# trzy/FasterRCNN

Hardware: AMD Instinct MI355X
Metric: images/sec (600x1000) Faster-RCNN VGG-16 inference (higher is better)
Workload: dtype f32 (float32 tensors and accumulation; 15 GEMM layers in the f32x3 split-operand emulation = two fp16 terms per block-scaled operand, three fp16 MFMAs per product; 0 in f32x6 = three bf16 terms, six bf16 MFMAs; the other 2 on exact-f32 MFMA; strict exact-f32 everywhere: config.strict_f32_images_per_

## Files before the change

### fasterrcnn_amd/_native.py

```python
import ctypes as C
import os

_HERE = os.path.dirname(os.path.abspath(__file__))
LIB_PATH = os.environ.get("FRCNN_LIB_PATH") or os.path.join(_HERE, "csrc", "libfrcnn_hip.so")

OK = 0
ABI_VERSION = 21
ERRORS = {0: "FRCNN_OK", -1: "FRCNN_EINVAL", -2: "FRCNN_EHIP", -3: "FRCNN_ENOMEM",
          -4: "FRCNN_EUNSUPPORTED", -5: "FRCNN_ENODEVICE"}
RELU = 1
POOL2 = 2
NUM_KCLASS = 11
KCLASS_NAMES = ("conv3x3_mfma", "conv3x3_c3", "linear_mfma", "proposals", "roi_pool", "other", "winograd_transforms",
                "winograd_gemm", "winograd_x6_transforms", "winograd_x6_gemm", "winograd_x3f")

SYMBOLS = (
    "frcnn_abi_version", "frcnn_error_string", "frcnn_last_hip_error", "frcnn_device_count",
    "frcnn_anchors", "frcnn_pack_conv3x3", "frcnn_pack_conv3x3_c3", "frcnn_pack_fc_chw_to_hwc",
    "frcnn_pack_stack_rows", "frcnn_conv3x3_c3", "frcnn_conv3x3_c3_cmax", "frcnn_conv3x3_workspace_bytes", "frcnn_conv3x3_nhwc",
    "frcnn_maxpool2x2_nhwc",
    "frcnn_linear_workspace_bytes", "frcnn_linear", "frcnn_softmax_rows", "frcnn_rpn_proposals",
    "frcnn_nms", "frcnn_roi_pool", "frcnn_roi_pool_x3t", "frcnn_detections", "frcnn_ctx_create", "frcnn_ctx_create_proposals", "frcnn_ctx_destroy",
    "frcnn_ctx_bytes", "frcnn_vgg16_forward", "frcnn_ctx_tensor", "frcnn_ctx_timing_enable",
    "frcnn_ctx_timing_read",
    "frcnn_fold_bn_pack", "frcnn_conv_workspace_bytes", "frcnn_conv_nhwc", "frcnn_conv_nhwc_math", "frcnn_conv_nhwc_x3g", "frcnn_conv_nhwc_x3g_tickets", "frcnn_pack_conv_x3g_weights", "frcnn_x3_saturation_events", "frcnn_tensor_absmax", "frcnn_conv7x7_s2_c3",
    "frcnn_maxpool3x3_s2_nhwc", "frcnn_spatial_mean_nhwc", "frcnn_resnet_forward", "frcnn_rpn_targets",
    "frcnn_preprocess_workspace_bytes", "frcnn_preprocess",
    "frcnn_conv3x3_uses_winograd", "frcnn_resnet_block_uses_winograd", "frcnn_pack_conv3x3_winograd",
    "frcnn_pack_conv3x3_winograd_taps", "frcnn_conv3x3_winograd_workspace_bytes",
    "frcnn_conv3x3_nhwc_winograd",
    "frcnn_conv3x3_uses_winograd_fused", "frcnn_resnet_block_uses_winograd_fused", "frcnn_pack_conv3x3_winograd_fused", "frcnn_pack_conv3x3_winograd_fused_taps",
    "frcnn_conv3x3_nhwc_winograd_fused",
    "frcnn_roi_align", "frcnn_roi_align_backward",
    "frcnn_x6t_record_bytes", "frcnn_split_rows_x6t", "frcnn_gemm_x6t_workspace_bytes", "frcnn_gemm_x6t", "frcnn_split_pixels_x6t", "frcnn_split_patches3x3_x6t",
    "frcnn_conv3x3_uses_winograd_x6", "frcnn_conv3x3_winograd_x6_pack_bytes", "frcnn_pack_conv3x3_winograd_x6",
    "frcnn_conv3x3_winograd_x6_workspace_bytes", "frcnn_conv3x3_nhwc_winograd_x6",
    "frcnn_pixel_absmax", "frcnn_split_pixels_x3t", "frcnn_split_patches3x3_x3t",
    "frcnn_x3t_blob_bytes", "frcnn_pack_rows_x3t", "frcnn_conv3x3_winograd_x3_pack_bytes", "frcnn_pack_conv3x3_winograd_x3",
    "frcnn_conv3x3_winograd_x3_workspace_bytes", "frcnn_conv3x3_nhwc_winograd_x3",
    "frcnn_conv3x3_winograd_x3_fused_workspace_bytes", "frcnn_conv3x3_nhwc_winograd_x3_fused", "frcnn_conv3x3_nhwc_winograd_x3_chain",
    "frcnn_x3t_record_bytes", "frcnn_rows_scale_x3t", "frcnn_split_rows_x3t", "frcnn_gemm_x3t_workspace_bytes", "frcnn_gemm_x3t",
    "frcnn_conv3x3_nhwc_winograd_fused_maps", "frcnn_ctx_create_backbone", "frcnn_resnet_backbone", "frcnn_resnet_forward_features", "frcnn_resnet_rpn_roipool", "frcnn_ctx_create_head", "frcnn_resnet_head",
    "frcnn_label_proposals", "frcnn_gather_rows", "frcnn_rpn_loss", "frcnn_detector_loss",
    "frcnn_gemm_tn_math", "frcnn_conv3x3_wgrad_math", "frcnn_conv_wgrad_math", "frcnn_bottleneck_backward_workspace_bytes", "frcnn_bottleneck_backward",
    "frcnn_gemm_tn_workspace_bytes", "frcnn_gemm_tn", "frcnn_conv3x3_wgrad_workspace_bytes", "frcnn_conv3x3_wgrad",
    "frcnn_pack_conv3x3_dgrad", "frcnn_relu_backward", "frcnn_dropout", "frcnn_dropout_relu_backward", "frcnn_add_inplace", "frcnn_maxpool2x2_backward",
    "frcnn_roi_pool_backward_workspace_bytes", "frcnn_roi_pool_backward", "frcnn_transpose", "frcnn_sgd_step", "frcnn_sgd_step_fold",
    "frcnn_conv_wgrad_workspace_bytes", "frcnn_conv_wgrad", "frcnn_conv_dgrad_workspace_bytes", "frcnn_conv_dgrad", "frcnn_conv_dgrad_math",
    "frcnn_pack_conv_dgrad", "frcnn_scale_rows", "frcnn_bn_scale_shift", "frcnn_spatial_mean_backward",
    "frcnn_ops_roi_align", "frcnn_ops_roi_align_backward", "frcnn_ops_roi_pool", "frcnn_ops_roi_pool_backward",
    "frcnn_ops_nms_workspace_bytes", "frcnn_ops_nms",
    "frcnn_ops_ms_roi_align", "frcnn_ops_ms_roi_align_workspace_bytes", "frcnn_ops_ms_roi_align_backward",
    "frcnn_ops_half_run", "frcnn_ops_roi_align_16", "frcnn_ops_roi_align_backward_16", "frcnn_ops_roi_pool_16",
    "frcnn_ops_roi_pool_backward_16", "frcnn_ops_ms_roi_align_16", "frcnn_ops_ms_roi_align_backward_16",
)


# ... 230 lines not shown
    "frcnn_detector_loss": (C.c_int, [_vp, _vp, _vp, _vp, _i, _i, _vp, _vp, _i, _vp]),
    "frcnn_gemm_tn_workspace_bytes": (C.c_size_t, [_i, _i, _i]),
    "frcnn_gemm_tn": (C.c_int, [_vp, _i, _vp, _i, _vp, _i, _i, _i, _i, _vp, _sz, _vp]),
    "frcnn_gemm_tn_math": (C.c_int, [_vp, _i, _vp, _i, _vp, _i, _i, _i, _i, _i, _vp, _sz, _vp]),
    "frcnn_conv3x3_wgrad_math": (C.c_int, [_vp, _vp, _vp, _i, _i, _i, _i, _i, _vp, _sz, _vp]),
    "frcnn_conv_wgrad_math": (C.c_int, [_vp, _vp, _vp, _i, _i, _i, _i, _i, _i, _i, _i, _i, _vp, _sz, _vp]),
    "frcnn_bottleneck_backward_workspace_bytes": (C.c_int, [_vp, _vp, _vp, _vp, _i, _i, _i, _i, _i, C.POINTER(C.c_size_t), C.POINTER(C.c_size_t)]),
    "frcnn_bottleneck_backward": (C.c_int, [_vp, _vp, _vp, _vp, _vp, _vp, _vp, _vp, _vp, _vp, _vp, _vp, _vp, _i, _i, _i, _i, _i, _i, _vp, _sz, _vp, _sz,
                                            _vp, _vp]),
    "frcnn_conv3x3_wgrad_workspace_bytes": (C.c_size_t, [_i, _i, _i, _i]),
    "frcnn_conv3x3_wgrad": (C.c_int, [_vp, _vp, _vp, _i, _i, _i, _i, _vp, _sz, _vp]),
    "frcnn_pack_conv3x3_dgrad": (C.c_int, [_vp, _vp, _i, _i, _vp]),
    "frcnn_conv_wgrad_workspace_bytes": (C.c_size_t, [_i] * 8),
    "frcnn_conv_wgrad": (C.c_int, [_vp, _vp, _vp, _i, _i, _i, _i, _i, _i, _i, _i, _vp, _sz, _vp]),
    "frcnn_conv_dgrad_workspace_bytes": (C.c_size_t, [_i] * 8),
    "frcnn_conv_dgrad": (C.c_int, [_vp, _vp, _vp, _vp, _i, _i, _i, _i, _i, _i, _i, _i, _vp, _sz, _vp]),
    "frcnn_conv_dgrad_math": (C.c_int, [_vp, _vp, _vp, _vp, _i, _i, _i, _i, _i, _i, _i, _i, _i, _vp, _sz, _vp]),
    "frcnn_pack_conv_dgrad": (C.c_int, [_vp, _vp, _i, _i, _i, _vp]),
    "frcnn_scale_rows": (C.c_int, [_vp, _vp, _vp, _i, _i, _i, _vp]),
    "frcnn_bn_scale_shift": (C.c_int, [_vp, _vp, _vp, _vp, _f, _i, _vp, _vp, _vp]),
    "frcnn_spatial_mean_backward": (C.c_int, [_vp, _vp, _i, _i, _i, _i, _vp]),
    "frcnn_relu_backward": (C.c_int, [_vp, _vp, _sz, _vp]),
    "frcnn_dropout": (C.c_int, [_vp, _sz, _f, _f, _vp, C.c_uint32, C.c_uint32, _vp, _vp]),
    "frcnn_dropout_relu_backward": (C.c_int, [_vp, _vp, _sz, _f, _vp]),
    "frcnn_add_inplace": (C.c_int, [_vp, _vp, _sz, _vp]),
    "frcnn_maxpool2x2_backward": (C.c_int, [_vp, _vp, _vp, _i, _i, _i, _vp]),
    "frcnn_roi_pool_backward_workspace_bytes": (C.c_size_t, [_i, _i, _i]),
    "frcnn_roi_pool_backward": (C.c_int, [_vp, _i, _i, _i, _vp, _i, _i, _f, _vp, _vp, _i, _vp, _sz, _vp]),
    "frcnn_transpose": (C.c_int, [_vp, _i, _vp, _i, _i, _i, _vp]),
    "frcnn_sgd_step": (C.c_int, [_vp, _vp, _vp, _sz, _f, _f, _f, _i, _vp]),
    "frcnn_sgd_step_fold": (C.c_int, [_vp, _vp, _vp, _sz, _f, _f, _f, _i, _vp, _vp, _i, _i, _vp]),
    "frcnn_ctx_timing_enable": (C.c_int, [_vp, _i]),
    "frcnn_ctx_timing_read": (C.c_int, [_vp, C.POINTER(C.c_double), C.POINTER(C.c_int64), _i]),
}


def lib():
    global _lib
    if _lib is not None:
        return _lib
    import torch
    if not os.path.exists(LIB_PATH):
        raise RuntimeError(
            "fasterrcnn_amd: %s is missing. Build it with `python -m fasterrcnn_amd.build` "
            "(hipcc --offload-arch=gfx950). There is no CPU fallback for this path." % LIB_PATH)
    try:
        handle = C.CDLL(LIB_PATH)
    except OSError as e:
        raise RuntimeError("fasterrcnn_amd: cannot load %s: %s" % (LIB_PATH, e)) from e
    for name in SYMBOLS:
        try:
            fn = getattr(handle, name)
        except AttributeError as e:
            raise RuntimeError("fasterrcnn_amd: %s does not export %s (stale build?)" % (LIB_PATH, name)) from e
        restype, argtypes = _SIGNATURES[name]
        fn.restype = restype
        fn.argtypes = argtypes
    if handle.frcnn_abi_version() != ABI_VERSION:
        raise RuntimeError("fasterrcnn_amd: ABI version mismatch in %s" % LIB_PATH)
    _lib = handle
    return _lib


def check(rc, where):
    if rc != OK:
        detail = ""
        if rc == -2:
# ... 30 lines not shown
```

### fasterrcnn_amd/csrc/api.hip

```cpp
#include "common.h"
#include <algorithm>
#include <cmath>
#include <cstring>
#include <string>
#include <vector>
#include <new>

namespace frcnn {

static thread_local std::string g_hip_error;
void set_hip_error(hipError_t e) { g_hip_error = hipGetErrorString(e); }

static size_t align_up(size_t v, size_t a) { return (v + a - 1) / a * a; }

struct EventRec { int cls; hipEvent_t start, stop; };

}

using namespace frcnn;

struct frcnn_ctx {
    int max_h = 0, max_w = 0, max_rois = 0, max_images = 0;
    int max_fh = 0, max_fw = 0, a_cap = 0, pre_cap = 0;
    void* slab = nullptr;
// ... 3 lines not shown
    float *rpn_trunk = nullptr;
    float *rpn_head = nullptr;
    float *scores = nullptr;
    int32_t* sorted_idx = nullptr;
    float *anchor_map = nullptr, *valid_map = nullptr;
    float *roi_out = nullptr;
    float *fc1_out = nullptr, *fc2_out = nullptr;
    void *roi_rec = nullptr, *fc1_rec = nullptr;
    int rec_rows = 0;
    float *roi_inv = nullptr, *fc1_inv = nullptr, *fm_cmax = nullptr;
    float *head_logits = nullptr;
    void* lin_ws = nullptr; size_t lin_ws_bytes = 0;
    void* conv_ws = nullptr; size_t conv_ws_bytes = 0;
    void* wino_ws = nullptr; size_t wino_ws_bytes = 0;
    void* wx_ws = nullptr; size_t wx_ws_bytes = 0;
    int max_head_rois = 0;
    float* x3f_cmax = nullptr; size_t x3f_cmax_bytes = 0;
    void* rx_rec = nullptr; size_t rx_rec_bytes = 0;
    void* rx_ws = nullptr; size_t rx_ws_bytes = 0;
    float* rx_aux = nullptr; size_t rx_aux_floats = 0;
    float* gx_max = nullptr; int gx_next = 0; const float* gx_x = nullptr;
    unsigned* gx_cnt = nullptr;
    float* res_buf[5] = {nullptr, nullptr, nullptr, nullptr, nullptr};
    size_t res_buf_floats = 0;
    int last_c = 512, last_vec = 4096, last_head_ld = 128;
    ProposalScratch ps{};
    int anc_h = -1, anc_w = -1, anc_fh = -1, anc_fw = -1;
    int last_fh = 0, last_fw = 0, last_pre = 0, last_post = 0;
    bool timing = false;
    std::vector<EventRec> recs;
    std::vector<hipEvent_t> free_events;
    double t_ms[FRCNN_NUM_KCLASS] = {0};
    int64_t t_cnt[FRCNN_NUM_KCLASS] = {0};
};

namespace {

struct Scope {
    frcnn_ctx* c; int cls; hipStream_t s; hipEvent_t e0 = nullptr, e1 = nullptr; bool on;
    Scope(frcnn_ctx* c_, int cls_, hipStream_t s_) : c(c_), cls(cls_), s(s_), on(c_ && c_->timing) {
        if (!on) return;
        e0 = take(); e1 = take();
        if (!e0 || !e1) { on = false; return; }
        (void)hipEventRecord(e0, s);
    }
    ~Scope() {
        if (!on) return;
        (void)hipEventRecord(e1, s);
        c->recs.push_back(EventRec{cls, e0, e1});
    }
    hipEvent_t take() {
        if (!c->free_events.empty()) { hipEvent_t e = c->free_events.back(); c->free_events.pop_back(); return e; }
        hipEvent_t e = nullptr;
        if (hipEventCreate(&e) != hipSuccess) return nullptr;
        return e;
    }
};

inline hipStream_t as_stream(void* s) { return reinterpret_cast<hipStream_t>(s); }

}

extern "C" {

int frcnn_abi_version(void) { return FRCNN_ABI_VERSION; }

// ... 899 lines not shown
    unsigned char* p = static_cast<unsigned char*>(c->slab);
    for (auto& it : items) { *it.p = p; p += align_up(it.bytes, 256); }
    c->lin_ws_bytes = lin;
    c->conv_ws_bytes = cws;
    proposal_scratch_carve(c->ps, ps_base, c->a_cap, c->pre_cap, 2048);
    *out = c;
    return FRCNN_OK;
}

int frcnn_ctx_create_proposals(frcnn_ctx** out, int max_image_h, int max_image_w)
{
    if (!out || max_image_h < 16 || max_image_w < 16) return FRCNN_EINVAL;
    frcnn_ctx* c = new (std::nothrow) frcnn_ctx();
    if (!c) return FRCNN_ENOMEM;
    c->max_h = max_image_h; c->max_w = max_image_w; c->max_rois = 0;
    c->max_fh = cdiv(max_image_h, 16); c->max_fw = cdiv(max_image_w, 16);
    c->a_cap = c->max_fh * c->max_fw * 9;
    if (c->a_cap < 16384) c->a_cap = 16384;
    c->pre_cap = 16384;
    const size_t total = align_up(proposal_scratch_bytes(c->a_cap, c->pre_cap, 2048), 256);
    hipError_t e = hipMalloc(&c->slab, total);
    if (e != hipSuccess) { set_hip_error(e); delete c; return FRCNN_ENOMEM; }
    c->slab_bytes = total;
    proposal_scratch_carve(c->ps, c->slab, c->a_cap, c->pre_cap, 2048);
    *out = c;
    return FRCNN_OK;
}

void frcnn_ctx_destroy(frcnn_ctx* ctx)
{
    if (!ctx) return;
    for (auto& r : ctx->recs) { (void)hipEventDestroy(r.start); (void)hipEventDestroy(r.stop); }
    for (auto e : ctx->free_events) (void)hipEventDestroy(e);
    if (ctx->slab) (void)hipFree(ctx->slab);
    if (ctx->wino_ws) (void)hipFree(ctx->wino_ws);
    if (ctx->wx_ws) (void)hipFree(ctx->wx_ws);
    if (ctx->x3f_cmax) (void)hipFree(ctx->x3f_cmax);
    if (ctx->roi_rec) (void)hipFree(ctx->roi_rec);
    if (ctx->rx_rec) (void)hipFree(ctx->rx_rec);
    if (ctx->rx_ws) (void)hipFree(ctx->rx_ws);
    if (ctx->rx_aux) (void)hipFree(ctx->rx_aux);
    if (ctx->gx_max) (void)hipFree(ctx->gx_max);
    if (ctx->gx_cnt) (void)hipFree(ctx->gx_cnt);
    delete ctx;
}

size_t frcnn_ctx_bytes(const frcnn_ctx* ctx) { return ctx ? ctx->slab_bytes + ctx->wino_ws_bytes + ctx->wx_ws_bytes + ctx->rx_rec_bytes + ctx->rx_ws_bytes + (ctx->roi_rec ? (size_t)ctx->rec_rows * (49 * 512 + 4096) * 6 : 0) : 0; }

int frcnn_ctx_timing_enable(frcnn_ctx* ctx, int enable)
{
    if (!ctx) return FRCNN_EINVAL;
    ctx->timing = enable != 0;
    return FRCNN_OK;
}

int frcnn_ctx_timing_read(frcnn_ctx* ctx, double ms[FRCNN_NUM_KCLASS], int64_t launches[FRCNN_NUM_KCLASS], int reset)
{
    if (!ctx || !ms || !launches) return FRCNN_EINVAL;
    for (auto& r : ctx->recs) {
        FRCNN_HIP_TRY(hipEventSynchronize(r.stop));
        float t = 0.f;
        FRCNN_HIP_TRY(hipEventElapsedTime(&t, r.start, r.stop));
        ctx->t_ms[r.cls] += t;
        ctx->t_cnt[r.cls] += 1;
        ctx->free_events.push_back(r.start);
        ctx->free_events.push_back(r.stop);
// ... 715 lines not shown
                const float* d_anchor_map, const float* d_valid_map, float* d_props, float* d_classes, float* d_deltas, int32_t* d_counts,
                hipStream_t s)
{
    int rc = resnet_rpn_roi(c, w, p, H, W, fh, fw, C, d_anchor_map, d_valid_map, d_props, d_counts, c->roi_out, s);
    if (rc) return rc;
    return resnet_head(c, w, p, c->roi_out, p->post_nms, d_classes, d_deltas, s);
}
}

int frcnn_resnet_forward(frcnn_ctx* c, const frcnn_resnet_weights* w, const frcnn_forward_params* p,
                         const float* d_image, int H, int W, const float* d_anchor_map,
                         const float* d_valid_map, float* d_props, float* d_classes, float* d_deltas,
                         int32_t* d_counts, void* stream)
{
    if (!c || !w || !p || !d_image || !d_props || !d_classes || !d_deltas || !d_counts) return FRCNN_EINVAL;
    if (H < 32 || W < 32 || H > c->max_h || W > c->max_w) return FRCNN_EINVAL;
    if (p->post_nms < 1 || p->post_nms > c->max_rois || p->pre_nms < 1 || p->pre_nms > c->pre_cap) return FRCNN_EINVAL;
    if (w->num_classes < 2 || w->num_classes > FRCNN_MAX_NUM_CLASSES) return FRCNN_EUNSUPPORTED;
    int rc = resnet_check_params(p);
    if (rc) return rc;
    rc = resnet_check_weights(w, true);
    if (rc) return rc;
    hipStream_t s = as_stream(stream);
    BlocksTargetScope target_scope(p->conv_blocks_target, p->winograd_tile_rows, p->x6_gemm_tiles);
    if (p->math_mode == FRCNN_MATH_F32_WINOGRAD) { rc = ensure_wino_ws(c); if (rc) return rc; }
    int cur = 0, fh = 0, fw = 0, C = 0;
    rc = resnet_stage1(c, w, p, d_image, 1, H, W, &cur, &fh, &fw, &C, s);
    if (rc) return rc;
    if (fh > c->max_fh || fw > c->max_fw || C > 1024 || C % 64) return FRCNN_EINVAL;
    FRCNN_HIP_TRY(hipMemcpyAsync(c->fm, c->res_buf[cur], (size_t)fh * fw * C * sizeof(float), hipMemcpyDeviceToDevice, s));
    return resnet_tail(c, w, p, H, W, fh, fw, C, d_anchor_map, d_valid_map, d_props, d_classes, d_deltas, d_counts, s);
}

int frcnn_ctx_create_backbone(frcnn_ctx** out, int max_image_h, int max_image_w, int max_images)
{
    if (!out || max_image_h < 32 || max_image_w < 32 || max_images < 1 || max_images > 64) return FRCNN_EINVAL;
    frcnn_ctx* c = new (std::nothrow) frcnn_ctx();
    if (!c) return FRCNN_ENOMEM;
    c->max_h = max_image_h; c->max_w = max_image_w; c->max_rois = 0; c->max_images = max_images;
    c->max_fh = cdiv(max_image_h, 16); c->max_fw = cdiv(max_image_w, 16);
    const size_t stem = (size_t)((max_image_h + 1) / 2) * ((max_image_w + 1) / 2) * 64;
    c->res_buf_floats = stem * max_images;
    const size_t cws = (size_t)160 << 20;
    const size_t total = 5 * align_up(c->res_buf_floats * 4, 256) + align_up(cws, 256);
    hipError_t e = hipMalloc(&c->slab, total);
    if (e != hipSuccess) { set_hip_error(e); delete c; return FRCNN_ENOMEM; }
    c->slab_bytes = total;
    unsigned char* q = static_cast<unsigned char*>(c->slab);
    for (int i = 0; i < 5; ++i) { c->res_buf[i] = reinterpret_cast<float*>(q); q += align_up(c->res_buf_floats * 4, 256); }
    c->conv_ws = q; c->conv_ws_bytes = cws;
    *out = c;
    return FRCNN_OK;
}

int frcnn_resnet_backbone(frcnn_ctx* c, const frcnn_resnet_weights* w, const frcnn_forward_params* p, const float* d_images,
                          int n_images, int H, int W, float* d_features, void* stream)
{
    if (!c || !w || !p || !d_images || !d_features || n_images < 1) return FRCNN_EINVAL;
    if (H < 32 || W < 32 || H > c->max_h || W > c->max_w || n_images > (c->max_images > 0 ? c->max_images : 1)) return FRCNN_EINVAL;
    int rc = resnet_check_params(p);
    if (rc) return rc;
    rc = resnet_check_weights(w, false);
    if (rc) return rc;
    hipStream_t s = as_stream(stream);
    BlocksTargetScope target_scope(p->conv_blocks_target, p->winograd_tile_rows, p->x6_gemm_tiles);
    int cur = 0, fh = 0, fw = 0, C = 0;
// ... 105 lines not shown
```

### fasterrcnn_amd/models/faster_rcnn.py

```python
import ctypes as C
from dataclasses import dataclass

import numpy as np
import torch as t
from torch import nn

from .. import _native as nv
from .. import runtime as rt
from .. import utils
from . import anchors
from . import detector
from . import resnet
from . import rpn
from . import vgg16


class Pending:
    def __init__(self, model, slot, with_detections):
        self._model, self._slot, self._with_detections = model, slot, with_detections
        self._result = None

    def result(self):
        if self._result is None:
            slot = self._slot
# ... 49 lines not shown
        self.max_proposals_post_nms = 300
        self.rpn_nms_threshold = 0.7
        self.rpn_min_side = 16.0
        self.detector_nms_threshold = 0.3
        self.inflight_conv_blocks_target = 320
        self.inflight_winograd_tile_rows = 128
        self.inflight_x6_gemm_tiles = 2

        self._math_mode = "f32"
        self.math_mode = "f32_winograd"
        self._x6_conv1x1 = "off"
        self.x6_conv1x1 = "head" if self._is_resnet else "off"
        self._x6_conv1x1_arith = "f32x6"
        self.x6_conv1x1_arith = "f32x3" if self._is_resnet else "f32x6"
        self._bottleneck_g3 = "off"
        if self._is_resnet and getattr(backbone, "architecture", None) == resnet.Architecture.ResNet50:
            self.bottleneck_g3 = "backbone"
        self._winograd_x6_layers = ()
        self.winograd_x6_layers = ("rpn_trunk",) if self._is_resnet else nv.DEFAULT_X6_LAYERS_VGG16
        self._fc_math_mode = "f32"
        self.fc_math_mode = "f32" if self._is_resnet else "f32x3"
        self._winograd_x3_layers = ()
        self.winograd_x3_layers = ("rpn_trunk",) if self._is_resnet else nv.DEFAULT_X3_LAYERS_VGG16
        self._winograd_x3f_layers = ()
        if not self._is_resnet:
            self.winograd_x3f_layers = nv.DEFAULT_X3F_LAYERS_VGG16
        self._inflight_winograd_x3f_layers = ()
        self._alone_winograd_x3f_layers = ()
        if not self._is_resnet:
            self.inflight_winograd_x3f_layers = nv.DEFAULT_INFLIGHT_X3F_LAYERS_VGG16
            self.alone_winograd_x3f_layers = nv.DEFAULT_ALONE_X3F_LAYERS_VGG16

        self.use_hip_graphs = False
        self.batch_head = False
        self._grad_math = "f32"
        self._train_state = None
        self._gradient_sync = None
        self._slots = {}
        self._lanes = {}
        self._wstruct = None
        self._wstruct_key = None
        self._wkeep = None

    @property
    def math_mode(self):
        return self._math_mode

    @math_mode.setter
    def math_mode(self, mode):
        if mode not in nv.MATH_MODES:
            raise ValueError("math_mode must be one of %s" % sorted(nv.MATH_MODES))
        self._math_mode = mode
        if getattr(self, "_train_state", None) is not None:
            self._train_state.winograd = mode == "f32_winograd"
        self._stage1_feature_extractor.math_mode = mode
        self._stage2_region_proposal_network.math_mode = mode
        if self._is_resnet:
            self._stage3_detector_network._pool_to_feature_vector.math_mode = mode

    @property
    def x6_conv1x1(self):
        return self._x6_conv1x1

    @x6_conv1x1.setter
    def x6_conv1x1(self, mode):
        mode = {False: "off", True: "all", None: "off"}.get(mode, mode)
# ... 446 lines not shown
        self._check_limits(with_detections=score_threshold is not None)
        self.sync_parameters()
        device = self._device()
        image = rt.as_f32_cuda(image_data, "image_data")
        if image.device != device:
            raise RuntimeError("image_data is on %s but the model is on %s" % (image.device, device))
        if image.dim() != 4 or image.shape[1] != 3:
            raise ValueError("image_data must be shaped (1, 3, H, W)")
        h, w = int(image.shape[2]), int(image.shape[3])
        slot = self._slot(slot_index, h, w, device)
        if slot.busy:
            raise RuntimeError("slot %d still has an un-collected image in flight" % slot_index)
        amap = rt.to_device_map(anchor_map, device)
        vmap = rt.to_device_map(anchor_valid_map, device)
        if amap is None or vmap is None:
            amap = vmap = None
        weights = self._weights()
        params = self._forward_params(slot_index)
        lib = nv.lib()
        with_det = score_threshold is not None
        fwd, fwd_name = ((lib.frcnn_resnet_forward, "frcnn_resnet_forward") if self._is_resnet
                         else (lib.frcnn_vgg16_forward, "frcnn_vgg16_forward"))

        def body(img, sp):
            nv.check(fwd(slot.ctx.handle, C.byref(weights), C.byref(params), nv.ptr(img), h, w,
                         nv.ptr(amap), nv.ptr(vmap), nv.ptr(slot.props), nv.ptr(slot.classes),
                         nv.ptr(slot.deltas), nv.ptr(slot.counts), sp), fwd_name)
            self._enqueue_outputs(slot, h, w, score_threshold, sp)

        gkey = None
        if self.use_hip_graphs and amap is None and not slot.ctx.timing:
            gkey = (h, w, None if score_threshold is None else float(score_threshold), float(self.detector_nms_threshold),
                    tuple(getattr(params, f) for f, _ in params._fields_), self._wstruct_key)
        with t.cuda.device(device):
            stream = slot.use_stream()
            if slot.stream is not None:
                stream.wait_stream(t.cuda.current_stream(device))
            if wait_event is not None:
                stream.wait_event(wait_event)
            with t.cuda.stream(stream):
                if gkey is not None and slot.graph_key == gkey and slot.graph is not None:
                    slot.graph_input.copy_(image)
                    slot.graph.replay()
                elif gkey is not None and slot.graph_key == gkey:
                    if slot.capture_stream is None:
                        slot.capture_stream = t.cuda.Stream(device=device)
                    slot.graph_input = t.empty_like(image)
                    slot.graph_input.copy_(image)
                    graph = t.cuda.CUDAGraph()
                    slot.capture_stream.wait_stream(stream)
                    with t.cuda.graph(graph, stream=slot.capture_stream, capture_error_mode="thread_local"):
                        body(slot.graph_input, t.cuda.current_stream(device).cuda_stream)
                    stream.wait_stream(slot.capture_stream)
                    slot.graph = graph
                    graph.replay()
                else:
                    slot.graph, slot.graph_input, slot.graph_key = None, None, gkey
                    body(image, stream.cuda_stream)
                slot.done.record(stream)
        slot.busy = True
        slot.keepalive = (image, amap, vmap)
        return Pending(self, slot, with_det)

    def forward(self, image_data, anchor_map=None, anchor_valid_map=None):
        with t.no_grad():
            return self._enqueue(image_data, anchor_map, anchor_valid_map, None, 0).result()

    @utils.no_grad
    def predict(self, image_data, score_threshold, anchor_map=None, anchor_valid_map=None):
        self.eval()
        assert image_data.shape[0] == 1, "Batch size must be 1"
        return self._enqueue(image_data, anchor_map, anchor_valid_map, score_threshold, 0).result()

    @utils.no_grad
    def predict_async(self, image_data, score_threshold, slot, anchor_map=None, anchor_valid_map=None, wait_event=None):
        return self._enqueue(image_data, anchor_map, anchor_valid_map, score_threshold, int(slot), wait_event)

    def forward_batch(self, image_data, lane=0):
        with t.no_grad():
            return [p.result() for p in self._enqueue_batch(image_data, None, lane)]

    @utils.no_grad
    def predict_batch(self, image_data, score_threshold, lane=0):
        self.eval()
        return [p.result() for p in self._enqueue_batch(image_data, score_threshold, lane)]

    @utils.no_grad
    def predict_batch_async(self, image_data, score_threshold, lane=0):
        return self._enqueue_batch(image_data, score_threshold, lane)

    def context(self, slot=0):
# ... 38 lines not shown
```

### fasterrcnn_amd/runtime.py

```python
import ctypes as C

import numpy as np
import torch as t

from . import _native as nv


class Context:
    def __init__(self, device, max_h, max_w, max_rois, proposals_only=False):
        nv.require_gpu()
        self.device = t.device(device)
        self.max_h, self.max_w, self.max_rois = int(max_h), int(max_w), 0 if proposals_only else int(max_rois)
        handle = C.c_void_p()
        with t.cuda.device(self.device):
            if proposals_only:
                nv.check(nv.lib().frcnn_ctx_create_proposals(C.byref(handle), self.max_h, self.max_w), "frcnn_ctx_create_proposals")
            else:
                nv.check(nv.lib().frcnn_ctx_create(C.byref(handle), self.max_h, self.max_w, self.max_rois),
                         "frcnn_ctx_create")
        self.handle = handle
        self.timing = False

    def fits(self, h, w, rois):
        return h <= self.max_h and w <= self.max_w and rois <= self.max_rois

    @property
    def nbytes(self):
        return int(nv.lib().frcnn_ctx_bytes(self.handle))

    def tensor(self, which, dtype=t.float32):
        p, n = C.c_void_p(), C.c_size_t()
        nv.check(nv.lib().frcnn_ctx_tensor(self.handle, which, C.byref(p), C.byref(n)), "frcnn_ctx_tensor")
        itemsize = t.empty((), dtype=dtype).element_size()
        out = t.empty((n.value // itemsize,), dtype=dtype, device=self.device)
        t.cuda.current_stream(self.device).synchronize()
        rc = _hip_memcpy_dtod(out.data_ptr(), p.value, n.value)
        if rc != 0:
            raise RuntimeError("hipMemcpy failed: %d" % rc)
        return out

    def timing_enable(self, on):
        self.timing = bool(on)
        nv.check(nv.lib().frcnn_ctx_timing_enable(self.handle, 1 if on else 0), "frcnn_ctx_timing_enable")

    def timing_read(self, reset=True):
        ms = (C.c_double * nv.NUM_KCLASS)()
        cnt = (C.c_int64 * nv.NUM_KCLASS)()
        nv.check(nv.lib().frcnn_ctx_timing_read(self.handle, ms, cnt, 1 if reset else 0), "frcnn_ctx_timing_read")
        return {nv.KCLASS_NAMES[i]: (ms[i], cnt[i]) for i in range(nv.NUM_KCLASS)}

    def __del__(self):
        try:
            if getattr(self, "handle", None) is not None and self.handle.value:
                nv.lib().frcnn_ctx_destroy(self.handle)
                self.handle = None
            if getattr(self, "head_handle", None) is not None and self.head_handle.value:
                nv.lib().frcnn_ctx_destroy(self.head_handle)
                self.head_handle = None
        except Exception:
            pass


_hip = None


def _hip_memcpy_dtod(dst, src, nbytes):
    global _hip
    if _hip is None:
        _hip = C.CDLL("libamdhip64.so")
        _hip.hipMemcpy.restype = C.c_int
        _hip.hipMemcpy.argtypes = [C.c_void_p, C.c_void_p, C.c_size_t, C.c_int]
    return _hip.hipMemcpy(dst, src, nbytes, 3)


_slot_streams = {}


def _lane_stream_index(lane, image):
    return 1 + (int(image) % 4)


def slot_stream(device, index):
    if isinstance(index, tuple) and len(index) == 3 and index[0] == "lane":
        index = _lane_stream_index(index[1], index[2])
    key = (str(t.device(device)), index)
    st = _slot_streams.get(key)
    if st is None:
        st = t.cuda.Stream(device=t.device(device))
        _slot_streams[key] = st
    return st


class Slot:
    def __init__(self, device, max_h, max_w, max_rois, num_classes, own_stream, index=None):
        self.device = t.device(device)
        self.ctx = Context(device, max_h, max_w, max_rois)
        self.max_rois, self.num_classes = int(max_rois), int(num_classes)
        self.stream = (slot_stream(self.device, index) if index is not None else t.cuda.Stream(device=self.device)) if own_stream else None
        nfg = num_classes - 1
        d = self.device
        self.props = t.zeros((max_rois, 4), dtype=t.float32, device=d)
        self.classes = t.zeros((max_rois, num_classes), dtype=t.float32, device=d)
        self.deltas = t.zeros((max_rois, nfg * 4), dtype=t.float32, device=d)
        self.counts = t.zeros((4,), dtype=t.int32, device=d)
        self.det = t.zeros((nfg, max_rois, 5), dtype=t.float64, device=d)
        self.det_cnt = t.zeros((nfg,), dtype=t.int32, device=d)
        self.h_det = t.zeros((nfg, max_rois, 5), dtype=t.float64).pin_memory()
        self.h_det_cnt = t.zeros((nfg,), dtype=t.int32).pin_memory()
        self.h_counts = t.zeros((4,), dtype=t.int32).pin_memory()
        self.done = t.cuda.Event()
        self.roi_ready = t.cuda.Event()
        self.graph, self.graph_key, self.graph_input, self.capture_stream = None, None, None, None
        self.busy = False
        self.keepalive = None

    def use_stream(self):
        return self.stream if self.stream is not None else t.cuda.current_stream(self.device)


class BackboneLane:
    def __init__(self, device, max_h, max_w, max_images, channels):
        nv.require_gpu()
        self.device = t.device(device)
        self.max_h, self.max_w, self.max_images = int(max_h), int(max_w), int(max_images)
        handle = C.c_void_p()
        with t.cuda.device(self.device):
            nv.check(nv.lib().frcnn_ctx_create_backbone(C.byref(handle), self.max_h, self.max_w, self.max_images), "frcnn_ctx_create_backbone")
            self.stream = t.cuda.Stream(device=self.device)
        self.handle = handle
        fh, fw = feature_map_shape(self.max_h, self.max_w)
        self.features = t.empty((self.max_images * fh * fw * int(channels),), dtype=t.float32, device=self.device)
        self.ready = t.cuda.Event()
        self.readers = []
        self.keepalive = None
        self.head_handle = None
        self.head_rois = 0
        self.roi_all = self.classes_all = self.deltas_all = None
        self.head_done = t.cuda.Event()

    def ensure_head(self, max_rois, num_classes, channels=1024):
        total = self.max_images * int(max_rois)
        if self.head_handle is not None and self.head_rois >= total and self.classes_all.shape[1] == num_classes:
            return
        if self.head_handle is not None:
            t.cuda.synchronize(self.device)
            nv.lib().frcnn_ctx_destroy(self.head_handle)
            self.head_handle = None
        handle = C.c_void_p()
        with t.cuda.device(self.device):
            nv.check(nv.lib().frcnn_ctx_create_head(C.byref(handle), total), "frcnn_ctx_create_head")
# ... 47 lines not shown
```

### include/frcnn_hip.h

```cpp
#ifndef FRCNN_HIP_H
#define FRCNN_HIP_H

#include <stddef.h>
#include <stdint.h>

#ifdef __cplusplus
extern "C" {
#endif

#define FRCNN_OK            0
#define FRCNN_EINVAL       -1
#define FRCNN_EHIP         -2
#define FRCNN_ENOMEM       -3
#define FRCNN_EUNSUPPORTED -4
#define FRCNN_ENODEVICE    -5

#define FRCNN_ABI_VERSION 21

#define FRCNN_RELU   1u
#define FRCNN_POOL2  2u
#define FRCNN_X3G_WSPLIT 0x800u

int         frcnn_abi_version(void);
const char* frcnn_error_string(int code);
// ... 242 lines not shown
    const float *wd, *bd;
    int32_t cin, width, cout, stride;
    int32_t x6_mask;
    int32_t x3_mask;
    const float* wmax;
    int32_t g3;
    int32_t reserved0;
} frcnn_bottleneck_weights;
#define FRCNN_X6_CONV1 1
#define FRCNN_X6_CONV3 2
#define FRCNN_X6_DOWN  4
#define FRCNN_X6_CONV2 8

typedef struct frcnn_resnet_weights {
    const float* stem_w;
    const float* stem_b;
    int32_t n_blocks[4];
    frcnn_bottleneck_weights blocks[FRCNN_RESNET_MAX_BLOCKS];
    const float* rpn_conv_w;
    const float* rpn_conv_b;
    const float* rpn_head_w;
    const float* rpn_head_b;
    const float* head_w;
    const float* head_b;
    int32_t num_classes;
} frcnn_resnet_weights;

int frcnn_resnet_forward(frcnn_ctx* ctx, const frcnn_resnet_weights* w, const frcnn_forward_params* p,
                         const float* d_image, int H, int W,
                         const float* d_anchor_map, const float* d_valid_map,
                         float* d_props, float* d_classes, float* d_deltas, int32_t* d_counts,
                         void* stream);

int frcnn_ctx_create_backbone(frcnn_ctx** out, int max_image_h, int max_image_w, int max_images);
int frcnn_resnet_backbone(frcnn_ctx* ctx, const frcnn_resnet_weights* w, const frcnn_forward_params* p,
                          const float* d_images, int n_images, int H, int W, float* d_features, void* stream);
int frcnn_resnet_forward_features(frcnn_ctx* ctx, const frcnn_resnet_weights* w, const frcnn_forward_params* p,
                                  const float* d_feature_map, int H, int W,
                                  const float* d_anchor_map, const float* d_valid_map,
                                  float* d_props, float* d_classes, float* d_deltas, int32_t* d_counts,
                                  void* stream);
int frcnn_resnet_rpn_roipool(frcnn_ctx* ctx, const frcnn_resnet_weights* w, const frcnn_forward_params* p, const float* d_feature_map, int H,
                             int W, const float* d_anchor_map, const float* d_valid_map, float* d_props, int32_t* d_counts, float* d_roi_out,
                             void* stream);
int frcnn_ctx_create_head(frcnn_ctx** out, int max_rois_total);
int frcnn_resnet_head(frcnn_ctx* ctx, const frcnn_resnet_weights* w, const frcnn_forward_params* p, float* d_rois, int n_rois, float* d_classes,
                      float* d_deltas, void* stream);


int frcnn_label_proposals(const float* d_props, const int32_t* d_n_props, int max_props,
                          const float* d_gt_boxes, const int32_t* d_gt_class_idx, int n_gt, int num_classes,
                          float min_background_iou, float min_object_iou,
                          const float box_delta_means[4], const float box_delta_stds[4],
                          float* d_out_props, int32_t* d_out_class_idx, float* d_out_gt_classes,
                          float* d_out_gt_box_deltas, int32_t* d_out_count, void* stream);

int frcnn_gather_rows(const float* d_src, const int32_t* d_idx, int n, int row_floats, float* d_dst, void* stream);

int frcnn_rpn_loss(const float* d_head, int ld_head, int cells, const int32_t* d_sample, int n_sample,
                   const float* d_rpn_map, float* d_losses, float* d_grad_head, void* stream);

int frcnn_detector_loss(const float* d_classes, const float* d_deltas, const float* d_gt_classes,
                        const float* d_gt_box_deltas, int n, int num_classes, float* d_losses,
                        float* d_grad_logits, int ld_grad, void* stream);

size_t frcnn_gemm_tn_workspace_bytes(int M, int N, int R);
// ... 90 lines not shown
```

Measured before the change: 854.4.

## Submit whole predict in one native call with packed output block

Adds a native submit entry point that runs the forward pass, runs detections and copies outputs back in one call, replacing several Python-side launches and copies. Counts, detection counts and detections now live in one contiguous device block that is copied to pinned host memory with a single async memcpy. Cross-stream dependencies skip the event wait when the producer stream is already idle and otherwise reuse a ring of events. New slot streams are probed so that two slots do not share one hardware queue. The gain in host overhead and overlap is small against GPU-bound inference, and the queue probe adds startup cost.

New measurement: 968.2, median of 6. 13.3% higher.

```diff
diff --git a/fasterrcnn_amd/_native.py b/fasterrcnn_amd/_native.py
--- a/fasterrcnn_amd/_native.py
+++ b/fasterrcnn_amd/_native.py
@@ -23,6 +23,7 @@
     "frcnn_nms", "frcnn_roi_pool", "frcnn_roi_pool_x3t", "frcnn_detections", "frcnn_ctx_create", "frcnn_ctx_create_proposals", "frcnn_ctx_destroy",
     "frcnn_ctx_bytes", "frcnn_vgg16_forward", "frcnn_ctx_tensor", "frcnn_ctx_timing_enable",
     "frcnn_ctx_timing_read",
+    "frcnn_output_block_layout", "frcnn_stream_depend", "frcnn_ctx_submit_stats", "frcnn_predict_submit", "frcnn_streams_share_queue",
     "frcnn_fold_bn_pack", "frcnn_conv_workspace_bytes", "frcnn_conv_nhwc", "frcnn_conv_nhwc_math", "frcnn_conv_nhwc_x3g", "frcnn_conv_nhwc_x3g_tickets", "frcnn_pack_conv_x3g_weights", "frcnn_x3_saturation_events", "frcnn_tensor_absmax", "frcnn_conv7x7_s2_c3",
     "frcnn_maxpool3x3_s2_nhwc", "frcnn_spatial_mean_nhwc", "frcnn_resnet_forward", "frcnn_rpn_targets",
     "frcnn_preprocess_workspace_bytes", "frcnn_preprocess",
@@ -319,7 +320,19 @@
     "frcnn_sgd_step_fold": (C.c_int, [_vp, _vp, _vp, _sz, _f, _f, _f, _i, _vp, _vp, _i, _i, _vp]),
     "frcnn_ctx_timing_enable": (C.c_int, [_vp, _i]),
     "frcnn_ctx_timing_read": (C.c_int, [_vp, C.POINTER(C.c_double), C.POINTER(C.c_int64), _i]),
+    "frcnn_output_block_layout": (C.c_int, [_i, _i, C.POINTER(C.c_size_t), C.POINTER(C.c_size_t)]),
+    "frcnn_stream_depend": (C.c_int, [_vp, _vp, _vp]),
+    "frcnn_streams_share_queue": (C.c_int, [_vp, _vp, C.POINTER(C.c_int)]),
+    "frcnn_ctx_submit_stats": (C.c_int, [_vp, C.POINTER(C.c_int64), C.POINTER(C.c_int64)]),
+    "frcnn_predict_submit": (C.c_int, [_vp, _i, _vp, C.POINTER(ForwardParams), _vp, _i, _i, _vp, _vp, _vp, _vp, _vp, _vp, _vp, _i,
+                                       _i, _f, _f, _i, _vp, _vp, _vp]),
 }
+
+
+def output_block_layout(max_rois, num_classes):
+    off, total = (C.c_size_t * 3)(), C.c_size_t()
+    check(lib().frcnn_output_block_layout(int(max_rois), int(num_classes), off, C.byref(total)), "frcnn_output_block_layout")
+    return int(off[0]), int(off[1]), int(off[2]), int(total.value)
 
 
 def lib():
diff --git a/fasterrcnn_amd/csrc/api.hip b/fasterrcnn_amd/csrc/api.hip
--- a/fasterrcnn_amd/csrc/api.hip
+++ b/fasterrcnn_amd/csrc/api.hip
@@ -59,6 +59,10 @@
     std::vector<hipEvent_t> free_events;
     double t_ms[FRCNN_NUM_KCLASS] = {0};
     int64_t t_cnt[FRCNN_NUM_KCLASS] = {0};
+    static constexpr int DEP_RING = 8;
+    hipEvent_t dep_ring[DEP_RING] = {nullptr};
+    unsigned dep_next = 0;
+    int64_t dep_taken = 0, dep_skipped = 0;
 };
 
 namespace {
@@ -1024,6 +1028,7 @@
     if (!ctx) return;
     for (auto& r : ctx->recs) { (void)hipEventDestroy(r.start); (void)hipEventDestroy(r.stop); }
     for (auto e : ctx->free_events) (void)hipEventDestroy(e);
+    for (auto e : ctx->dep_ring) if (e) (void)hipEventDestroy(e);
     if (ctx->slab) (void)hipFree(ctx->slab);
     if (ctx->wino_ws) (void)hipFree(ctx->wino_ws);
     if (ctx->wx_ws) (void)hipFree(ctx->wx_ws);
@@ -1805,6 +1810,106 @@
     return resnet_tail(c, w, p, H, W, fh, fw, C, d_anchor_map, d_valid_map, d_props, d_classes, d_deltas, d_counts, s);
 }
 
+int frcnn_output_block_layout(int max_rois, int ncls, size_t offsets[3], size_t* total_bytes)
+{
+    if (!offsets || !total_bytes || max_rois < 1 || ncls < 2 || ncls > FRCNN_MAX_NUM_CLASSES) return FRCNN_EINVAL;
+    const size_t nfg = (size_t)ncls - 1;
+    offsets[FRCNN_OUT_COUNTS] = 0;
+    offsets[FRCNN_OUT_DET_CNT] = align_up(4 * sizeof(int32_t), 16);
+    offsets[FRCNN_OUT_DET] = align_up(offsets[FRCNN_OUT_DET_CNT] + nfg * sizeof(int32_t), 16);
+    *total_bytes = align_up(offsets[FRCNN_OUT_DET] + nfg * (size_t)max_rois * 5 * sizeof(double), 16);
+    return FRCNN_OK;
+}
+
+__global__ void queue_probe_wait_kernel(long long ticks)
+{
+    const long long t0 = wall_clock64();
+    for (unsigned n = 0; n < (1u << 20) && wall_clock64() - t0 < ticks; ++n) { }
+}
+
+int frcnn_streams_share_queue(void* stream_a, void* stream_b, int* shared)
+{
+    if (!shared || stream_a == stream_b) return FRCNN_EINVAL;
+    hipStream_t a = as_stream(stream_a), b = as_stream(stream_b);
+    hipEvent_t ev[3] = {nullptr, nullptr, nullptr};
+    float ta = 0.f, tb = 0.f;
+    auto run = [&]() -> hipError_t {
+        hipError_t e;
+        for (auto& x : ev) if ((e = hipEventCreate(&x)) != hipSuccess) return e;
+        if ((e = hipEventRecord(ev[1], a)) != hipSuccess || (e = hipEventRecord(ev[2], b)) != hipSuccess) return e;
+        if ((e = hipStreamSynchronize(a)) != hipSuccess || (e = hipStreamSynchronize(b)) != hipSuccess) return e;
+        if ((e = hipEventRecord(ev[0], a)) != hipSuccess) return e;
+        queue_probe_wait_kernel<<<1, 1, 0, a>>>(20000);
+        if ((e = hipGetLastError()) != hipSuccess) return e;
+        if ((e = hipEventRecord(ev[1], a)) != hipSuccess || (e = hipEventRecord(ev[2], b)) != hipSuccess) return e;
+        if ((e = hipEventSynchronize(ev[1])) != hipSuccess || (e = hipEventSynchronize(ev[2])) != hipSuccess) return e;
+        if ((e = hipEventElapsedTime(&ta, ev[0], ev[1])) != hipSuccess) return e;
+        return hipEventElapsedTime(&tb, ev[0], ev[2]);
+    };
+    const hipError_t e = run();
+    for (auto x : ev) if (x) (void)hipEventDestroy(x);
+    if (e != hipSuccess) { (void)hipGetLastError(); set_hip_error(e); return FRCNN_EHIP; }
+    *shared = tb > 0.5f * ta ? 1 : 0;
+    return FRCNN_OK;
+}
+
+int frcnn_stream_depend(frcnn_ctx* c, void* producer, void* stream)
+{
+    if (!c) return FRCNN_EINVAL;
+    if (producer == stream) return FRCNN_OK;
+    const hipError_t q = hipStreamQuery(as_stream(producer));
+    if (q == hipSuccess) { ++c->dep_skipped; return FRCNN_OK; }
+    (void)hipGetLastError();
+    if (q != hipErrorNotReady) { set_hip_error(q); return FRCNN_EHIP; }
+    hipEvent_t& ev = c->dep_ring[c->dep_next++ % frcnn_ctx::DEP_RING];
+    if (!ev) FRCNN_HIP_TRY(hipEventCreateWithFlags(&ev, hipEventDisableTiming));
+    FRCNN_HIP_TRY(hipEventRecord(ev, as_stream(producer)));
+    FRCNN_HIP_TRY(hipStreamWaitEvent(as_stream(stream), ev, 0));
+    ++c->dep_taken;
+    return FRCNN_OK;
+}
+
+int frcnn_ctx_submit_stats(const frcnn_ctx* c, int64_t* taken, int64_t* skipped)
+{
+    if (!c || !taken || !skipped) return FRCNN_EINVAL;
+    *taken = c->dep_taken; *skipped = c->dep_skipped;
+    return FRCNN_OK;
+}
+
+int frcnn_predict_submit(frcnn_ctx* c, int backbone, const void* weights, const frcnn_forward_params* p,
+                         const float* d_image, int H, int W, const float* d_anchor_map, const float* d_valid_map,
+                         float* d_props, float* d_classes, float* d_deltas, void* d_block, void* h_block, int max_rois,
+                         int with_detections, float score_threshold, float nms_threshold,
+                         int depend, void* producer, void* stream, void* done_event)
+{
+    if (!c || !weights || !p || !d_block || !h_block || (backbone != 0 && backbone != 1)) return FRCNN_EINVAL;
+    const int ncls = backbone == 0 ? static_cast<const frcnn_vgg16_weights*>(weights)->num_classes
+                                   : static_cast<const frcnn_resnet_weights*>(weights)->num_classes;
+    size_t off[3], total = 0;
+    int rc = frcnn_output_block_layout(max_rois, ncls, off, &total);
+    if (rc) return rc;
+    if (p->post_nms > max_rois || max_rois > 512) return FRCNN_EINVAL;
+    unsigned char* db = static_cast<unsigned char*>(d_block);
+    int32_t* d_counts = reinterpret_cast<int32_t*>(db + off[FRCNN_OUT_COUNTS]);
+    if (depend) { rc = frcnn_stream_depend(c, producer, stream); if (rc) return rc; }
+    rc = backbone == 0
+        ? frcnn_vgg16_forward(c, static_cast<const frcnn_vgg16_weights*>(weights), p, d_image, H, W, d_anchor_map, d_valid_map,
+                              d_props, d_classes, d_deltas, d_counts, stream)
+        : frcnn_resnet_forward(c, static_cast<const frcnn_resnet_weights*>(weights), p, d_image, H, W, d_anchor_map, d_valid_map,
+                               d_props, d_classes, d_deltas, d_counts, stream);
+    if (rc) return rc;
+    size_t copy_bytes = off[FRCNN_OUT_DET_CNT];
+    if (with_detections) {
+        rc = frcnn_detections(d_props, d_classes, d_deltas, d_counts + 2, max_rois, ncls, H, W, score_threshold, nms_threshold,
+                              reinterpret_cast<double*>(db + off[FRCNN_OUT_DET]), reinterpret_cast<int32_t*>(db + off[FRCNN_OUT_DET_CNT]), stream);
+        if (rc) return rc;
+        copy_bytes = total;
+    }
+    FRCNN_HIP_TRY(hipMemcpyAsync(h_block, d_block, copy_bytes, hipMemcpyDeviceToHost, as_stream(stream)));
+    if (done_event) FRCNN_HIP_TRY(hipEventRecord(reinterpret_cast<hipEvent_t>(done_event), as_stream(stream)));
+    return FRCNN_OK;
+}
+
 int frcnn_ctx_create_backbone(frcnn_ctx** out, int max_image_h, int max_image_w, int max_images)
 {
     if (!out || max_image_h < 32 || max_image_w < 32 || max_images < 1 || max_images > 64) return FRCNN_EINVAL;
diff --git a/fasterrcnn_amd/models/faster_rcnn.py b/fasterrcnn_amd/models/faster_rcnn.py
--- a/fasterrcnn_amd/models/faster_rcnn.py
+++ b/fasterrcnn_amd/models/faster_rcnn.py
@@ -105,6 +105,7 @@
             self.alone_winograd_x3f_layers = nv.DEFAULT_ALONE_X3F_LAYERS_VGG16
 
         self.use_hip_graphs = False
+        self.native_submit = True
         self.batch_head = False
         self._grad_math = "f32"
         self._train_state = None
@@ -617,10 +618,32 @@
         if self.use_hip_graphs and amap is None and not slot.ctx.timing:
             gkey = (h, w, None if score_threshold is None else float(score_threshold), float(self.detector_nms_threshold),
                     tuple(getattr(params, f) for f, _ in params._fields_), self._wstruct_key)
+        native = bool(self.native_submit)
+        backbone_id = 1 if self._is_resnet else 0
+
+        def submit(img, sp, depend, producer, done_event):
+            nv.check(lib.frcnn_predict_submit(slot.ctx.handle, backbone_id, C.byref(weights), C.byref(params), nv.ptr(img), h, w,
+                                              nv.ptr(amap), nv.ptr(vmap), nv.ptr(slot.props), nv.ptr(slot.classes), nv.ptr(slot.deltas),
+                                              nv.ptr(slot.block), nv.ptr(slot.h_block), slot.max_rois, 1 if with_det else 0,
+                                              float(score_threshold) if with_det else 0.0, float(self.detector_nms_threshold),
+                                              1 if depend else 0, producer, sp, done_event), "frcnn_predict_submit")
+
         with t.cuda.device(device):
             stream = slot.use_stream()
+            producer = t.cuda.current_stream(device)
+            if native and gkey is None:
+                if wait_event is not None:
+                    stream.wait_event(wait_event)
+                submit(image, stream.cuda_stream, slot.stream is not None, producer.cuda_stream, slot.done.cuda_event)
+                slot.graph, slot.graph_input, slot.graph_key = None, None, None
+                slot.busy = True
+                slot.keepalive = (image, amap, vmap)
+                return Pending(self, slot, with_det)
             if slot.stream is not None:
-                stream.wait_stream(t.cuda.current_stream(device))
+                if native:
+                    nv.check(lib.frcnn_stream_depend(slot.ctx.handle, producer.cuda_stream, stream.cuda_stream), "frcnn_stream_depend")
+                else:
+                    stream.wait_stream(producer)
             if wait_event is not None:
                 stream.wait_event(wait_event)
             with t.cuda.stream(stream):
@@ -635,13 +658,19 @@
                     graph = t.cuda.CUDAGraph()
                     slot.capture_stream.wait_stream(stream)
                     with t.cuda.graph(graph, stream=slot.capture_stream, capture_error_mode="thread_local"):
-                        body(slot.graph_input, t.cuda.current_stream(device).cuda_stream)
+                        if native:
+                            submit(slot.graph_input, t.cuda.current_stream(device).cuda_stream, False, None, None)
+                        else:
+                            body(slot.graph_input, t.cuda.current_stream(device).cuda_stream)
                     stream.wait_stream(slot.capture_stream)
                     slot.graph = graph
                     graph.replay()
                 else:
                     slot.graph, slot.graph_input, slot.graph_key = None, None, gkey
-                    body(image, stream.cuda_stream)
+                    if native:
+                        submit(image, stream.cuda_stream, False, None, None)
+                    else:
+                        body(image, stream.cuda_stream)
                 slot.done.record(stream)
         slot.busy = True
         slot.keepalive = (image, amap, vmap)
diff --git a/fasterrcnn_amd/runtime.py b/fasterrcnn_amd/runtime.py
--- a/fasterrcnn_amd/runtime.py
+++ b/fasterrcnn_amd/runtime.py
@@ -49,6 +49,11 @@
         nv.check(nv.lib().frcnn_ctx_timing_read(self.handle, ms, cnt, 1 if reset else 0), "frcnn_ctx_timing_read")
         return {nv.KCLASS_NAMES[i]: (ms[i], cnt[i]) for i in range(nv.NUM_KCLASS)}
 
+    def submit_stats(self):
+        taken, skipped = C.c_int64(), C.c_int64()
+        nv.check(nv.lib().frcnn_ctx_submit_stats(self.handle, C.byref(taken), C.byref(skipped)), "frcnn_ctx_submit_stats")
+        return int(taken.value), int(skipped.value)
+
     def __del__(self):
         try:
             if getattr(self, "handle", None) is not None and self.handle.value:
@@ -86,9 +91,31 @@
     key = (str(t.device(device)), index)
     st = _slot_streams.get(key)
     if st is None:
-        st = t.cuda.Stream(device=t.device(device))
+        st = _new_slot_stream(t.device(device), [s for (d, _), s in _slot_streams.items() if d == key[0]])
         _slot_streams[key] = st
     return st
+
+
+_SLOT_STREAM_TRIES = 8
+_passed_over_streams = []
+
+
+def streams_share_queue(a, b):
+    shared = C.c_int(0)
+    with t.cuda.device(a.device):
+        nv.check(nv.lib().frcnn_streams_share_queue(a.cuda_stream, b.cuda_stream, C.byref(shared)), "frcnn_streams_share_queue")
+    return bool(shared.value)
+
+
+def _new_slot_stream(device, others):
+    first = None
+    for _ in range(_SLOT_STREAM_TRIES):
+        st = t.cuda.Stream(device=device)
+        if not any(o.cuda_stream == st.cuda_stream or (streams_share_queue(o, st) and streams_share_queue(st, o)) for o in others):
+            return st
+        _passed_over_streams.append(st)
+        first = first or st
+    return first
 
 
 class Slot:
@@ -102,13 +129,14 @@
         self.props = t.zeros((max_rois, 4), dtype=t.float32, device=d)
         self.classes = t.zeros((max_rois, num_classes), dtype=t.float32, device=d)
         self.deltas = t.zeros((max_rois, nfg * 4), dtype=t.float32, device=d)
-        self.counts = t.zeros((4,), dtype=t.int32, device=d)
-        self.det = t.zeros((nfg, max_rois, 5), dtype=t.float64, device=d)
-        self.det_cnt = t.zeros((nfg,), dtype=t.int32, device=d)
-        self.h_det = t.zeros((nfg, max_rois, 5), dtype=t.float64).pin_memory()
-        self.h_det_cnt = t.zeros((nfg,), dtype=t.int32).pin_memory()
-        self.h_counts = t.zeros((4,), dtype=t.int32).pin_memory()
+        o_counts, o_cnt, o_det, total = nv.output_block_layout(max_rois, num_classes)
+        self.block = t.zeros((total,), dtype=t.uint8, device=d)
+        self.h_block = t.zeros((total,), dtype=t.uint8).pin_memory()
+        self.counts, self.det_cnt, self.det = block_views(self.block, (o_counts, o_cnt, o_det), max_rois, num_classes)
+        self.h_counts, self.h_det_cnt, self.h_det = block_views(self.h_block, (o_counts, o_cnt, o_det), max_rois, num_classes)
         self.done = t.cuda.Event()
+        with t.cuda.device(d):
+            self.done.record(t.cuda.current_stream(d))
         self.roi_ready = t.cuda.Event()
         self.graph, self.graph_key, self.graph_input, self.capture_stream = None, None, None, None
         self.busy = False
@@ -116,6 +144,14 @@
 
     def use_stream(self):
         return self.stream if self.stream is not None else t.cuda.current_stream(self.device)
+
+
+def block_views(block, offsets, max_rois, num_classes):
+    nfg = int(num_classes) - 1
+    o_counts, o_cnt, o_det = offsets
+    return (block[o_counts:o_counts + 16].view(t.int32),
+            block[o_cnt:o_cnt + 4 * nfg].view(t.int32),
+            block[o_det:o_det + 40 * nfg * int(max_rois)].view(t.float64).view(nfg, int(max_rois), 5))
 
 
 class BackboneLane:
diff --git a/include/frcnn_hip.h b/include/frcnn_hip.h
--- a/include/frcnn_hip.h
+++ b/include/frcnn_hip.h
@@ -298,6 +298,23 @@
                          float* d_props, float* d_classes, float* d_deltas, int32_t* d_counts,
                          void* stream);
 
+#define FRCNN_OUT_COUNTS  0
+#define FRCNN_OUT_DET_CNT 1
+#define FRCNN_OUT_DET     2
+int frcnn_output_block_layout(int max_rois, int ncls, size_t offsets[3], size_t* total_bytes);
+
+int frcnn_streams_share_queue(void* stream_a, void* stream_b, int* shared);
+
+int frcnn_stream_depend(frcnn_ctx* ctx, void* producer, void* stream);
+
+int frcnn_ctx_submit_stats(const frcnn_ctx* ctx, int64_t* taken, int64_t* skipped);
+
+int frcnn_predict_submit(frcnn_ctx* ctx, int backbone, const void* weights, const frcnn_forward_params* p,
+                         const float* d_image, int H, int W, const float* d_anchor_map, const float* d_valid_map,
+                         float* d_props, float* d_classes, float* d_deltas, void* d_block, void* h_block, int max_rois,
+                         int with_detections, float score_threshold, float nms_threshold,
+                         int depend, void* producer, void* stream, void* done_event);
+
 int frcnn_ctx_create_backbone(frcnn_ctx** out, int max_image_h, int max_image_w, int max_images);
 int frcnn_resnet_backbone(frcnn_ctx* ctx, const frcnn_resnet_weights* w, const frcnn_forward_params* p,
                           const float* d_images, int n_images, int H, int W, float* d_features, void* stream);
```
